# NoelShin/PixelPick

Hardware: AMD Instinct MI355X
Metric: train_step_throughput (higher is better)
Workload: dtype f32; 1 GPU; BASELINE configs[1]: Cityscapes 256x512, C=19, DeepLabv3+-MobileNetV2; train step per-GPU batch 4 with 20 labelled px/img + Adam; acquisition entropy top-k=20, B=256 images/launch/GPU, NCHW fp32 logits; global_batch=4

## Files before the change

### include/pixelpick_hip.h

```cpp
#ifndef PIXELPICK_HIP_H
#define PIXELPICK_HIP_H

#include <stddef.h>
#include <stdint.h>

#ifdef __cplusplus
extern "C" {
#endif

typedef void* pp_stream_t;

enum {
    PP_OK = 0,
    PP_ERR_BAD_ARG = -1,
    PP_ERR_BAD_K = -2,
    PP_ERR_WORKSPACE = -3,
    PP_ERR_UNSUPPORTED = -4,
    PP_ERR_LAUNCH = -5
};

enum { PP_ACQ_ENTROPY = 0, PP_ACQ_LEAST_CONFIDENCE = 1, PP_ACQ_MARGIN = 2 };
enum { PP_ACQ_BALD = 3 };
#define PP_ACQ_REFERENCE_ORDER 0x100

// ... 244 lines not shown

int pp_bn_eval_affine(int C, const float* gamma, const float* beta, const float* running_mean, const float* running_var,
                      float eps, float* scale, float* shift, pp_stream_t stream);

int pp_scale_shift_act(const float* x, int64_t ldx, int64_t M, int C, const float* scale, const float* shift,
                       const float* residual, int64_t ldr, int act, float* y, int64_t ldy, pp_stream_t stream);

int pp_bn_bwd(const float* x, int64_t ldx, const float* dy, int64_t lddy, const float* y_act, int64_t ldya, int act,
              int64_t M, int C, const float* mean, const float* invstd, const float* gamma, float* dgamma, float* dbeta,
              float* dx, int64_t lddx, float* dres, int64_t lddr, void* workspace, size_t ws_bytes, pp_stream_t stream);

int pp_dwconv3x3_fwd(const float* x, int64_t ldx, int B, int H, int W, int C, const float* w, int stride, int pad, int dil,
                     float* y, int64_t ldy, pp_stream_t stream);

int pp_dwconv3x3_fwd_bn_act(const float* x, int64_t ldx, int B, int H, int W, int C, const float* w, int stride, int pad,
                            int dil, const float* gamma, const float* beta, const float* running_mean,
                            const float* running_var, float eps, const float* residual, int64_t ldr, int act, float* y,
                            int64_t ldy, pp_stream_t stream);
int pp_dwconv3x3_bwd_data(const float* dy, int64_t lddy, int B, int H, int W, int C, const float* w, int stride, int pad,
                          int dil, float* dx, int64_t lddx, pp_stream_t stream);
int pp_dwconv3x3_bwd_weight(const float* x, int64_t ldx, int B, int H, int W, int C, const float* dy, int64_t lddy,
                            int stride, int pad, int dil, float* dw, void* workspace, size_t ws_bytes, pp_stream_t stream);

size_t pp_groupnorm_workspace_bytes(int B, int64_t P, int C);
int pp_groupnorm_relu_fwd(const float* x, int64_t ldx, int B, int64_t P, int C, int G, const float* gamma, const float* beta,
                          float eps, int relu, float* y, int64_t ldy, float* mean, float* rstd, void* workspace,
                          size_t ws_bytes, pp_stream_t stream);
int pp_groupnorm_relu_bwd(const float* x, int64_t ldx, const float* dy, int64_t lddy, const float* y, int64_t ldy, int B,
                          int64_t P, int C, int G, const float* mean, const float* rstd, const float* gamma, float* dgamma,
                          float* dbeta, float* dx, int64_t lddx, void* workspace, size_t ws_bytes, pp_stream_t stream);

int pp_maxpool2d_fwd(const float* x, int64_t ldx, int B, int H, int W, int C, int ksize, int stride, int pad, float* y,
                     int64_t ldy, unsigned char* argmax, pp_stream_t stream);
int pp_maxpool2d_bwd(const float* dy, int64_t lddy, const unsigned char* argmax, int B, int H, int W, int C, int ksize, int stride,
                     int pad, float* dx, int64_t lddx, pp_stream_t stream);

int pp_pad2d(const float* x, int64_t ldx, int B, int H, int W, int C, int pad_top, int pad_left, int Hp, int Wp, float* y,
             int64_t ldy, pp_stream_t stream);
int pp_crop2d_add(const float* xp, int64_t ldxp, int B, int Hp, int Wp, int C, int pad_top, int pad_left, const float* add,
                  int64_t ldadd, float* y, int64_t ldy, int H, int W, pp_stream_t stream);

int pp_bilinear_fwd(const float* x, int64_t ldx, int B, int H, int W, int C, float* y, int64_t ldy, int Ho, int Wo,
                    int align_corners, float scale_h, float scale_w, int out_nchw, pp_stream_t stream);
size_t pp_bilinear_bwd_workspace_bytes(int B, int Ho, int W, int C);
int pp_bilinear_bwd(const float* dy, int64_t lddy, int B, int Ho, int Wo, int C, float* dx, int64_t lddx, int H, int W,
                    int align_corners, float scale_h, float scale_w, int dy_nchw, void* workspace, size_t ws_bytes,
// ... 91 lines not shown
```

### include/pixelpick_hip_knobs.h

```cpp
#ifndef PIXELPICK_HIP_KNOBS_H
#define PIXELPICK_HIP_KNOBS_H

void pp_debug_set_reduce_mode(int mode);
void pp_debug_set_exact_formula(int on);
void pp_debug_set_acq_tuning(int occ, int ppt);
void pp_debug_set_dw_variant(int v);
void pp_debug_set_splitk(int v);
void pp_debug_set_wgrad_target(int blocks);
void pp_debug_set_bn_target(int blocks);
void pp_debug_set_bn_bytes_per_block(int bytes);
void pp_debug_set_bn_probe(void* device_buffer);
void pp_debug_set_lsel_probe(void* device_buffer);
void pp_debug_set_conv_thresholds(int v);
void pp_debug_conv_plan(int64_t M, int Cn, int Ck, int ntaps, int* out4);
void pp_debug_set_conv_rows(int bits);
void pp_debug_set_conv_bn_fuse(int bits);
void pp_debug_set_x3_variant(int v);
void pp_debug_set_gemm_pw(int v);
void pp_debug_set_x3f(int v);
void pp_debug_set_x3(int on);
void pp_debug_set_conv_variant(int v);
void pp_debug_set_ce_stream(int on);
int pp_debug_launch_log(char* buf, int n);


int pp_debug_occupy_cus(int blocks, const int* stop, uint64_t max_ticks, uint64_t* started, pp_stream_t stream);


#endif
```

### pixelpick_amd/_lib.py

```python
import ctypes
import os
import struct

import torch

_HERE = os.path.dirname(os.path.abspath(__file__))
LIB_PATH = os.path.join(_HERE, "libpixelpick_hip.so")
KNOBS_LIB_PATH = os.path.join(_HERE, "libpixelpick_hip_knobs.so")
_use_knobs = [os.environ.get("PIXELPICK_KNOBS_BUILD", "0") not in ("", "0")]


def use_knobs_build(on: bool = True):
    if _lib is not None and _use_knobs[0] != bool(on):
        raise PixelPickHipError("use_knobs_build() after the library was loaded")
    _use_knobs[0] = bool(on)


def knobs_build() -> bool:
    return _use_knobs[0]

_i64, _p, _int, _sz, _f = ctypes.c_int64, ctypes.c_void_p, ctypes.c_int, ctypes.c_size_t, ctypes.c_float
_u64 = ctypes.c_uint64

SIGNATURES = {
# ... 66 lines not shown
    "pp_conv2d_bwd_weight_pre": (_int, [_p, _i64, _int, _int, _int, _int, _p, _i64, _int, _int, _int, _int, _int, _int, _p, _p, _p, _sz, _p, _p, _p]),
    "pp_conv2d_bwd_weight_partials": (_int, [_p, _i64, _int, _int, _int, _int, _p, _i64, _int, _int, _int, _int, _int, _int, _p, _p, _p, _sz, _p, _p]),
    "pp_wgrad_reduce_batch": (_int, [_p, _int, _p]),
    "pp_colreduce_workspace_bytes": (_sz, [_i64, _int]),
    "pp_bn_train_fwd": (_int, [_p, _i64, _i64, _int, _p, _p, _f, _f, _p, _p, _p, _p, _p, _p, _p, _sz, _p]),
    "pp_bn_eval_affine": (_int, [_int, _p, _p, _p, _p, _f, _p, _p, _p]),
    "pp_scale_shift_act": (_int, [_p, _i64, _i64, _int, _p, _p, _p, _i64, _int, _p, _i64, _p]),
    "pp_bn_bwd": (_int, [_p, _i64, _p, _i64, _p, _i64, _int, _i64, _int, _p, _p, _p, _p, _p, _p, _i64, _p, _i64, _p, _sz, _p]),
    "pp_bn_fused_workspace_bytes": (_sz, [_i64, _int]),
    "pp_bn_fused_sync_ints": (_sz, [_int]),
    "pp_bn_fused_rows_cached": (_int, [_i64, _int]),
    "pp_bn_train_fwd_fused": (_int, [_p, _i64, _i64, _int, _p, _p, _f, _f, _p, _p, _p, _p, _p, _i64, _int, _f, _u64, _p, _p, _i64, _p, _sz, _p, _sz, _p]),
    "pp_dwconv3x3_bn_train_fwd_fused": (_int, [_p, _i64, _int, _int, _int, _int, _p, _int, _int, _int, _p, _i64, _p, _p, _f, _f, _p, _p, _p, _p,
                                               _p, _i64, _int, _p, _i64, _p, _sz, _p, _sz, _p]),
    "pp_bn_bwd_fused": (_int, [_p, _i64, _p, _i64, _p, _i64, _int, _i64, _int, _p, _p, _p, _p, _p, _p, _i64, _p, _i64, _f, _p, _p, _sz, _p, _sz, _p]),
    "pp_bn_bwd_fused_sparse": (_int, [_p, _i64, _p, _i64, _p, _i64, _int, _i64, _int, _p, _p, _p, _p, _p, _p, _i64, _p, _i64, _f, _p, _p, _sz, _p, _sz, _p, _p]),
    "pp_row_flags": (_int, [_p, _i64, _i64, _int, _p, _p]),
    "pp_conv1x1_bwd_weight_sparse_workspace_bytes": (_sz, [_i64, _int, _int]),
    "pp_conv1x1_bwd_weight_sparse": (_int, [_p, _i64, _i64, _int, _p, _i64, _int, _p, _p, _p, _p, _sz, _p]),
    "pp_conv1x1_bwd_data_sparse": (_int, [_p, _i64, _i64, _int, _p, _int, _p, _p, _i64, _p]),
    "pp_dwconv3x3_fwd": (_int, [_p, _i64, _int, _int, _int, _int, _p, _int, _int, _int, _p, _i64, _p]),
    "pp_dwconv3x3_bwd_data": (_int, [_p, _i64, _int, _int, _int, _int, _p, _int, _int, _int, _p, _i64, _p]),
    "pp_dwconv3x3_bwd_weight": (_int, [_p, _i64, _int, _int, _int, _int, _p, _i64, _int, _int, _int, _p, _p, _sz, _p]),
    "pp_dwconv3x3_bwd_weight_partials": (_int, [_p, _i64, _int, _int, _int, _int, _p, _i64, _int, _int, _int, _p, _p, _sz, _p, _p]),
    "pp_groupnorm_workspace_bytes": (_sz, [_int, _i64, _int]),
    "pp_groupnorm_relu_fwd": (_int, [_p, _i64, _int, _i64, _int, _int, _p, _p, _f, _int, _p, _i64, _p, _p, _p, _sz, _p]),
    "pp_groupnorm_relu_bwd": (_int, [_p, _i64, _p, _i64, _p, _i64, _int, _i64, _int, _int, _p, _p, _p, _p, _p, _p, _i64, _p, _sz, _p]),
    "pp_maxpool2d_fwd": (_int, [_p, _i64, _int, _int, _int, _int, _int, _int, _int, _p, _i64, _p, _p]),
    "pp_maxpool2d_bwd": (_int, [_p, _i64, _p, _int, _int, _int, _int, _int, _int, _int, _p, _i64, _p]),
    "pp_pad2d": (_int, [_p, _i64, _int, _int, _int, _int, _int, _int, _int, _int, _p, _i64, _p]),
    "pp_crop2d_add": (_int, [_p, _i64, _int, _int, _int, _int, _int, _int, _p, _i64, _p, _i64, _int, _int, _p]),
    "pp_bilinear_fwd": (_int, [_p, _i64, _int, _int, _int, _int, _p, _i64, _int, _int, _int, _f, _f, _int, _p]),
    "pp_bilinear_bwd_workspace_bytes": (_sz, [_int] * 4),
    "pp_bilinear_bwd": (_int, [_p, _i64, _int, _int, _int, _int, _p, _i64, _int, _int, _int, _f, _f, _int, _p, _sz, _p]),
    "pp_image_colsum": (_int, [_p, _i64, _int, _i64, _int, _f, _p, _i64, _p]),
    "pp_image_broadcast": (_int, [_p, _i64, _int, _i64, _int, _f, _p, _i64, _p]),
    "pp_dropout": (_int, [_p, _i64, _p, _i64, _i64, _int, _f, ctypes.c_uint64, _p, _p]),
    "pp_dropout2d": (_int, [_p, _i64, _p, _i64, _int, _i64, _int, _f, ctypes.c_uint64, _p, _p]),
    "pp_aug_resample_h": (_int, [_p, _int, _int, _p, _p, _int, _int, _p, _p]),
    "pp_aug_vcrop": (_int, [_p, _p, _p] + [_int] * 11 + [_p, _p]),
    "pp_aug_labels": (_int, [_p, _p, _int, _p, _p, _p, _p] + [_int] * 8 + [_p, _p, _p]),
    "pp_aug_jitter": (_int, [_p, _i64, _int, _f, _p, _p]),
    "pp_aug_blur": (_int, [_p, _int, _int, _p, _int, _p, _p]),
    "pp_aug_blur_q8": (_int, [_p, _int, _int, _p, _int, _p, _p]),
    "pp_aug_to_tensor": (_int, [_p, _i64, ctypes.POINTER(_f), ctypes.POINTER(_f), _p, _p]),
    "pp_sparse_ce_workspace_bytes": (_sz, []),
# ... 16 lines not shown
    "pp_set_kernel_events": (None, [_p, _p, _int]),
    "pp_set_comm_cu_reserve": (None, [_int]),
    "pp_get_comm_cu_reserve": (_int, []),
    "pp_plan_create": (_p, []),
    "pp_plan_destroy": (None, [_p]),
    "pp_plan_size": (_i64, [_p]),
    "pp_plan_entry_args": (_int, [_p]),
    "pp_plan_add_call": (_int, [_p, _p, _p, _int]),
    "pp_plan_add_event_record": (_int, [_p, _p, _p]),
    "pp_plan_add_stream_wait": (_int, [_p, _p, _p]),
    "pp_plan_add_join": (_int, [_p, _p, _p]),
    "pp_plan_add_host_break": (_int, [_p]),
    "pp_plan_replay": (_int, [_p, _i64, ctypes.POINTER(_i64)]),
}

KNOB_SIGNATURES = {
    "pp_debug_set_reduce_mode": (None, [_int]),
    "pp_debug_set_exact_formula": (None, [_int]),
    "pp_debug_set_acq_tuning": (None, [_int, _int]),
    "pp_debug_set_dw_variant": (None, [_int]),
    "pp_debug_set_splitk": (None, [_int]),
    "pp_debug_set_wgrad_target": (None, [_int]),
    "pp_debug_set_bn_target": (None, [_int]),
    "pp_debug_set_bn_bytes_per_block": (None, [_int]),
    "pp_debug_set_bn_probe": (None, [_p]),
    "pp_debug_set_lsel_probe": (None, [_p]),
    "pp_debug_set_conv_thresholds": (None, [_int]),
    "pp_debug_conv_plan": (None, [_i64, _int, _int, _int, _p]),
    "pp_debug_set_conv_variant": (None, [_int]),
    "pp_debug_set_ce_stream": (None, [_int]),
    "pp_debug_set_conv_rows": (None, [_int]),
    "pp_debug_set_conv_bn_fuse": (None, [_int]),
    "pp_debug_set_x3": (None, [_int]),
    "pp_debug_set_x3f": (None, [_int]),
    "pp_debug_set_gemm_pw": (None, [_int]),
    "pp_debug_set_x3_variant": (None, [_int]),
    "pp_debug_occupy_cus": (_int, [_int, _p, _u64, _p, _p]),
    "pp_debug_launch_log": (_int, [ctypes.c_char_p, _int]),
}

_lib = None
knob_epoch = [0]


def _knob_setter(fn):
    def setter(*args):
# ... 293 lines not shown
```

### pixelpick_amd/csrc/nn_ops.hip

```cpp
#include "pp_common.h"
#include "bn_xchg.h"
#include "lowres_tile.h"

namespace pp {

constexpr int kT = 256;

__device__ __forceinline__ float act_fwd(float z, int act)
{
    if (act == 1) return fmaxf(z, 0.0f);
    if (act == 2) return fminf(fmaxf(z, 0.0f), 6.0f);
    return z;
}
__device__ __forceinline__ void decode_bhwq(int64_t e, int cq, int Wd, int Hd, int& q, int& w, int& h, int& b)
{
    if (e <= 0xFFFFFFFFll) {
        const unsigned u = (unsigned)e;
        const unsigned t = u / (unsigned)cq;
        q = (int)(u - t * (unsigned)cq);
        const unsigned t2 = t / (unsigned)Wd;
        w = (int)(t - t2 * (unsigned)Wd);
        const unsigned t3 = t2 / (unsigned)Hd;
        h = (int)(t2 - t3 * (unsigned)Hd);
        b = (int)t3;
// ... 1107 lines not shown
                const int ih = 2 * ph + dr - pad, iw = 2 * pw + dc - pad;
                if ((unsigned)ih >= (unsigned)H || (unsigned)iw >= (unsigned)W) continue;
                float4 acc = make_float4(0.f, 0.f, 0.f, 0.f);
#pragma unroll
                for (int a = 0; a < 2; ++a) {
                    const int th = dr + 2 * a;
                    if (th > 2) continue;
                    const bool rok = (unsigned)(ph - a) < (unsigned)Ho;
#pragma unroll
                    for (int c = 0; c < 2; ++c) {
                        const int tw = dc + 2 * c;
                        if (tw > 2) continue;
                        if (!rok || (unsigned)(pw - c) >= (unsigned)Wo) continue;
                        const float4 gv = g[a][c], wv = ww[th * 3 + tw];
                        acc.x = fmaf(gv.x, wv.x, acc.x); acc.y = fmaf(gv.y, wv.y, acc.y);
                        acc.z = fmaf(gv.z, wv.z, acc.z); acc.w = fmaf(gv.w, wv.w, acc.w);
                    }
                }
                *reinterpret_cast<float4*>(dx + (((int64_t)b * H + ih) * W + iw) * lddx + q * 4) = acc;
            }
    }
}

__global__ __launch_bounds__(kT) void dwconv_bwd_weight_kernel(const float* x, int64_t ldx, int B, int H, int W, int cq,
                                                              const float* dy, int64_t lddy, int Ho, int Wo, int stride,
                                                              int pad, int dil, ColReduceGeom g, float* part,
                                                              const float* in_scale, const float* in_shift, int in_act)
{
    __shared__ float4 sh[kT];
    const int C = cq * 4;
    const int t = threadIdx.x;
    const int ql = t % g.cq_blk, ry = t / g.cq_blk;
    const int q = blockIdx.y * g.cq_blk + ql;
    const bool active = ry < g.rows_per_pass && q < cq;
    const int64_t M = (int64_t)B * Ho * Wo;
    float4 acc[9];
#pragma unroll
    for (int k = 0; k < 9; ++k) acc[k] = make_float4(0.f, 0.f, 0.f, 0.f);
    if (active) {
        const bool aff = in_scale != nullptr;
        float4 sc = make_float4(1.f, 1.f, 1.f, 1.f), sf = make_float4(0.f, 0.f, 0.f, 0.f);
        if (aff) { sc = *reinterpret_cast<const float4*>(in_scale + q * 4); sf = *reinterpret_cast<const float4*>(in_shift + q * 4); }
        const int64_t r0 = (int64_t)blockIdx.x * g.rows_per_block;
        const int64_t r1 = r0 + g.rows_per_block < M ? r0 + g.rows_per_block : M;
        for (int64_t r = r0 + ry; r < r1; r += g.rows_per_pass) {
            const unsigned ru = (unsigned)r;
// ... 901 lines not shown
        const float4 u = *reinterpret_cast<const float4*>(a + oa), v = *reinterpret_cast<const float4*>(b + ob);
        *reinterpret_cast<float4*>(y + oy) = make_float4(u.x + v.x, u.y + v.y, u.z + v.z, u.w + v.w);
    }
}

__global__ __launch_bounds__(kT) void nhwc_to_nchw_kernel(const float* x, int64_t ldx, int B, int C, int64_t HW, float* y)
{
    const int64_t total = (int64_t)B * C * HW;
    for (int64_t e = (int64_t)blockIdx.x * kT + threadIdx.x; e < total; e += (int64_t)gridDim.x * kT) {
        const int64_t pix = e % HW;
        const int64_t t = e / HW;
        const int c = (int)(t % C);
        const int64_t b = t / C;
        y[e] = x[(b * HW + pix) * ldx + c];
    }
}

static int g_ce_stream = 0;
static int g_bil_sep = 1;
static int g_dw_wgrad_x4 = 1, g_dw_wgrad_x4_blocks = 256;
static int g_dw_wgrad_cq_blk = 0, g_dw_wgrad_passes = 0;
static int g_dw_x4 = 1;
static int g_dw_s2 = 1;

static inline unsigned grid_for(int64_t total)
{
    int64_t b = cdiv(total, kT);
    if (b > 8192) b = 8192;
    if (b < 1) b = 1;
    return (unsigned)b;
}

static int need_c4(int C, const char* what)
{
    if (C < 4 || C % 4 != 0) return fail(PP_ERR_UNSUPPORTED, "%s: C=%d must be a positive multiple of 4", what, C);
    return PP_OK;
}

}

using namespace pp;

extern "C" {

#ifdef PP_DEBUG_KNOBS
void pp_debug_set_dw_variant(int v)
{
    g_dw_x4 = (v & 1) ? 0 : 1;
    g_dw_s2 = (v & 1048576) ? 0 : 1;
    g_bil_sep = (v & 256) ? 0 : 1;
    g_dw_wgrad_x4 = (v & 512) ? 0 : 1;
    { const int s4 = (v >> 10) & 7; g_dw_wgrad_x4_blocks = s4 == 1 ? 128 : s4 == 2 ? 512 : s4 == 3 ? 1024 : s4 == 4 ? 64 : 256; }
    { const int cb = (v >> 13) & 7; g_dw_wgrad_cq_blk = cb == 1 ? 8 : cb == 2 ? 16 : cb == 3 ? 32 : cb == 4 ? 64 : cb == 5 ? 128 : cb == 6 ? kT : 0; }
    { const int mp = (v >> 16) & 3; g_dw_wgrad_passes = mp == 1 ? 1 : mp == 2 ? 2 : mp == 3 ? 4 : 0; }
    const int sel = (v >> 1) & 7;
    g_dw_wgrad_blocks = sel == 1 ? 512 : sel == 2 ? 256 : sel == 3 ? 128 : sel == 4 ? 2048 : 1024;
}
#endif
#ifdef PP_DEBUG_KNOBS
void pp_debug_set_bn_target(int blocks) { g_bn_target_blocks = blocks > 0 ? (blocks > 1024 ? 1024 : blocks) : 0; }
#endif
#ifdef PP_DEBUG_KNOBS
void pp_debug_set_bn_bytes_per_block(int bytes)
{
    g_bn_bytes_per_block = bytes > 0 ? bytes : 0;
    g_bn_row_cache = bytes == -1 ? 0 : 1;
}
#endif
#ifdef PP_DEBUG_KNOBS
void pp_debug_set_ce_stream(int on) { g_ce_stream = on ? 1 : 0; }
#endif
static thread_local unsigned long long* g_bn_probe = nullptr;
#ifdef PP_DEBUG_KNOBS
void pp_debug_set_bn_probe(void* device_buffer) { g_bn_probe = reinterpret_cast<unsigned long long*>(device_buffer); }
#endif
int pp_bn_fused_capacity(void) { return bn_fused_capacity(); }

size_t pp_colreduce_workspace_bytes(int64_t M, int C)
{
    if (M < 1 || C < 4) return 256;
    ColReduceGeom g = col_geom(M, C);
    size_t a = (size_t)g.nblk_rows * 2 * C * 4;
    size_t b = (size_t)(M < 2048 ? M : 2048) * 9 * C * 4;
// ... 399 lines not shown
{
    if (!dy || !w || !dx) return fail(PP_ERR_BAD_ARG, "dwconv bwd_data: null");
    if (int rc = need_c4(C, "dwconv bwd_data")) return rc;
    const int Ho = (H + 2 * pad - 2 * dil - 1) / stride + 1, Wo = (W + 2 * pad - 2 * dil - 1) / stride + 1;
    if (stride == 1 && dil == 1 && g_dw_x4) {
        hipLaunchKernelGGL((dwconv_s1_x4_kernel<true>), dim3(grid_for((int64_t)B * H * ((W + 3) / 4) * (C / 4))), dim3(kT), 0,
                           as_stream(stream), dy, lddy, B, Ho, Wo, C / 4, w, 2 - pad, dx, lddx, H, W, Epilogue{});
        return check_launch("dwconv_s1_x4_kernel");
    }
    if (stride == 1 && dil == 2 && g_dw_x4) {
        hipLaunchKernelGGL((dwconv_s1_x4_kernel<true, 2>), dim3(grid_for((int64_t)B * H * ((W + 3) / 4) * (C / 4))), dim3(kT), 0,
                           as_stream(stream), dy, lddy, B, Ho, Wo, C / 4, w, 4 - pad, dx, lddx, H, W, Epilogue{});
        return check_launch("dwconv_s1_x4_kernel<2>");
    }
    if (stride == 2 && dil == 1 && pad >= 0 && pad <= 2 && g_dw_s2) {
        const int64_t items = (int64_t)B * ((H + pad + 1) / 2 + 1) * ((W + pad + 1) / 2 + 1) * (C / 4);
        hipLaunchKernelGGL(dwconv_s2_bwd_data_kernel, dim3(grid_for(items)), dim3(kT), 0, as_stream(stream), dy, lddy, B, Ho, Wo, C / 4, w, pad,
                           dx, lddx, H, W);
        return check_launch("dwconv_s2_bwd_data_kernel");
    }
    hipLaunchKernelGGL(dwconv_bwd_data_kernel, dim3(grid_for((int64_t)B * H * W * (C / 4))), dim3(kT), 0, as_stream(stream),
                       dy, lddy, B, Ho, Wo, C / 4, w, stride, pad, dil, dx, lddx, H, W);
    return check_launch("dwconv_bwd_data_kernel");
}

static int dwconv_bwd_weight_impl(const float* x, int64_t ldx, int B, int H, int W, int C, const float* dy, int64_t lddy,
                                  int stride, int pad, int dil, float* dw, void* workspace, size_t ws_bytes, pp_stream_t stream,
                                  const float* in_scale, const float* in_shift, int in_act, pp_reduce_job* job = nullptr)
{
    if (job) job->kind = 0;
    if (!x || !dy || !dw) return fail(PP_ERR_BAD_ARG, "dwconv bwd_weight: null");
    if (int rc = need_c4(C, "dwconv bwd_weight")) return rc;
    const int Ho = (H + 2 * pad - 2 * dil - 1) / stride + 1, Wo = (W + 2 * pad - 2 * dil - 1) / stride + 1;
    const int64_t M = (int64_t)B * Ho * Wo;
    if (M > 0x7FFFFFFFll) return fail(PP_ERR_UNSUPPORTED, "dwconv bwd_weight: more than 2^31 output pixels");
    if (!workspace || ws_bytes < pp_colreduce_workspace_bytes(M, C)) return fail(PP_ERR_WORKSPACE, "dwconv bwd_weight: workspace");
    const int cq_blk = g_dw_wgrad_cq_blk ? g_dw_wgrad_cq_blk : (M <= 8192 ? 32 : kT);
    const int passes = g_dw_wgrad_passes ? g_dw_wgrad_passes : (M <= 8192 ? 1 : 4);
    hipStream_t st = as_stream(stream);
    float* part = reinterpret_cast<float*>(workspace);
    if (stride == 1 && dil == 1 && Wo % 4 == 0 && g_dw_wgrad_x4) {
        ColReduceGeom g4 = col_geom(M / 4, C, g_dw_wgrad_x4_blocks, cq_blk, passes);
        if (g4.nblk_rows <= 2048) {
            hipLaunchKernelGGL(dwconv_bwd_weight_x4_kernel, dim3(g4.nblk_rows, g4.nblk_cols), dim3(kT), 0, st, x, ldx, B, H, W, C / 4,
                               dy, lddy, Ho, Wo, pad, g4, part, in_scale, in_shift, in_act);
            if (int rc = check_launch("dwconv_bwd_weight_x4_kernel")) return rc;
// ... 440 lines not shown
```

### pixelpick_amd/csrc/plan.hip

```cpp
#include "pp_common.h"

#include <cstring>
#include <type_traits>
#include <utility>
#include <vector>

namespace pp {
namespace {

template <typename T>
inline T unpack_slot(uint64_t s)
{
    if constexpr (std::is_same_v<T, float>) {
        float f;
        uint32_t lo = (uint32_t)s;
        memcpy(&f, &lo, 4);
        return f;
    } else if constexpr (std::is_same_v<T, double>) {
        double d;
        memcpy(&d, &s, 8);
        return d;
    } else if constexpr (std::is_pointer_v<T>) {
        return reinterpret_cast<T>(static_cast<uintptr_t>(s));
    } else {
// ... 57 lines not shown
    PP_PLAN_ENTRY(pp_x3_split),
    PP_PLAN_ENTRY(pp_conv2d_fwd_pre),
    PP_PLAN_ENTRY(pp_conv2d_bwd_data_pre),
    PP_PLAN_ENTRY(pp_conv2d_bwd_data_multi),
    PP_PLAN_ENTRY(pp_conv2d_fwd_pre2),
    PP_PLAN_ENTRY(pp_conv2d_bwd_data_pre2),
    PP_PLAN_ENTRY(pp_x3_split_weights),
    PP_PLAN_ENTRY(pp_conv2d_bwd_weight_pre),
    PP_PLAN_ENTRY(pp_conv2d_bwd_weight_partials),
    PP_PLAN_ENTRY(pp_wgrad_reduce_batch),
    PP_PLAN_ENTRY(pp_bn_train_fwd),
    PP_PLAN_ENTRY(pp_bn_eval_affine),
    PP_PLAN_ENTRY(pp_scale_shift_act),
    PP_PLAN_ENTRY(pp_bn_bwd),
    PP_PLAN_ENTRY(pp_bn_train_fwd_fused),
    PP_PLAN_ENTRY(pp_dwconv3x3_bn_train_fwd_fused),
    PP_PLAN_ENTRY(pp_bn_bwd_fused),
    PP_PLAN_ENTRY(pp_bn_bwd_fused_sparse),
    PP_PLAN_ENTRY(pp_row_flags),
    PP_PLAN_ENTRY(pp_conv1x1_bwd_weight_sparse),
    PP_PLAN_ENTRY(pp_conv1x1_bwd_data_sparse),
    PP_PLAN_ENTRY(pp_dwconv3x3_fwd),
    PP_PLAN_ENTRY(pp_dwconv3x3_bwd_data),
    PP_PLAN_ENTRY(pp_dwconv3x3_bwd_weight),
    PP_PLAN_ENTRY(pp_dwconv3x3_bwd_weight_partials),
    PP_PLAN_ENTRY(pp_groupnorm_relu_fwd),
    PP_PLAN_ENTRY(pp_groupnorm_relu_bwd),
    PP_PLAN_ENTRY(pp_maxpool2d_fwd),
    PP_PLAN_ENTRY(pp_maxpool2d_bwd),
    PP_PLAN_ENTRY(pp_pad2d),
    PP_PLAN_ENTRY(pp_crop2d_add),
    PP_PLAN_ENTRY(pp_bilinear_fwd),
    PP_PLAN_ENTRY(pp_bilinear_bwd),
    PP_PLAN_ENTRY(pp_image_colsum),
    PP_PLAN_ENTRY(pp_image_broadcast),
    PP_PLAN_ENTRY(pp_dropout),
    PP_PLAN_ENTRY(pp_dropout2d),
    PP_PLAN_ENTRY(pp_aug_resample_h),
    PP_PLAN_ENTRY(pp_aug_vcrop),
    PP_PLAN_ENTRY(pp_aug_labels),
    PP_PLAN_ENTRY(pp_aug_jitter),
    PP_PLAN_ENTRY(pp_aug_blur),
    PP_PLAN_ENTRY(pp_aug_blur_q8),
    PP_PLAN_ENTRY(pp_aug_to_tensor),
    PP_PLAN_ENTRY(pp_sparse_ce_fwd_bwd),
    PP_PLAN_ENTRY(pp_sparse_ce_lowres_fwd_bwd),
// ... 151 lines not shown
```

### pixelpick_amd/engine.py

```python
import contextlib
import math
import ctypes
import os
import weakref
from typing import List, Optional, Sequence

import torch

from . import _lib

ACT_NONE, ACT_RELU, ACT_RELU6 = 0, 1, 2


class Var:
    __slots__ = ("_t", "grad", "needs_grad", "_pending", "_lazy", "_bn_bwd_ctx", "_closed", "_grad_dst")

    def __init__(self, t: Optional[torch.Tensor], needs_grad: bool = True):
        self._t = t
        self.grad: Optional[torch.Tensor] = None
        self.needs_grad = needs_grad
        self._pending = None
        self._lazy = None
        self._bn_bwd_ctx = None
        self._closed = False
# ... 936 lines not shown
        if lazy_in is not None:
            raw, scale, shift, act = lazy_in
            with tape.side_stream_for(raw, dy, dw):
                ws = _ws(_wsbytes("pp_colreduce_workspace_bytes", B * Ho * Wo, C), dev)
                rc = L.pp_dwconv3x3_bwd_weight_affine_in(raw.data_ptr(), ldx, B, H, W, C, scale.data_ptr(), shift.data_ptr(), act,
                                                         dy.data_ptr(), lddy, stride, pad, dil, dw.data_ptr(), ws.data_ptr(), ws.numel(),
                                                         _stream())
            _lib.check(rc, "pp_dwconv3x3_bwd_weight_affine_in")
        else:
            with tape.side_stream_for(x.t, dy, dw):
                nws = _wsbytes("pp_colreduce_workspace_bytes", B * Ho * Wo, C)
                slot = tape.defer_slot(nws, dev)
                if slot is not None:
                    job, wptr, _ = slot
                    rc = L.pp_dwconv3x3_bwd_weight_partials(x.t.data_ptr(), ldx, B, H, W, C, dy.data_ptr(), lddy, stride, pad, dil,
                                                            dw.data_ptr(), wptr, nws, ctypes.addressof(job), _stream())
                    tape.defer_commit(job)
                else:
                    ws = _ws(nws, dev)
                    rc = L.pp_dwconv3x3_bwd_weight(x.t.data_ptr(), ldx, B, H, W, C, dy.data_ptr(), lddy, stride, pad, dil, dw.data_ptr(),
                                                   ws.data_ptr(), ws.numel(), _stream())
            _lib.check(rc, "pp_dwconv3x3_bwd_weight")
        tape.set_param_grad(w, dw)
    if x.needs_grad:
        dx = torch.empty((B, H, W, C), dtype=torch.float32, device=dev)
        rc = L.pp_dwconv3x3_bwd_data(dy.data_ptr(), lddy, B, H, W, C, w.data_ptr(), stride, pad, dil, dx.data_ptr(), C, _stream())
        _lib.check(rc, "pp_dwconv3x3_bwd_data")
        _acc(x, dx)


def _dw_bn_train_fused(tape: Tape, x: Var, gamma, beta, running_mean, running_var, act, residual, eps, momentum, dst):
    _, xin, w, _, stride, pad, dil = x._pending
    B, H, W, C, ld_in = _geom(xin.t)
    Ho, Wo = out_size(H, 3, stride, pad, dil), out_size(W, 3, stride, pad, dil)
    M = B * Ho * Wo
    if M > _BN_FUSED_MAXM or M >= (1 << 31) or C > 65536 or C % 4 or ld_in % 4:
        return None
    dev = xin.t.device
    xbuf = torch.empty((B, Ho, Wo, C), dtype=torch.float32, device=dev)
    mean = torch.empty(C, dtype=torch.float32, device=dev)
    invstd = torch.empty(C, dtype=torch.float32, device=dev)
    y = dst if dst is not None else torch.empty((B, Ho, Wo, C), dtype=torch.float32, device=dev)
    _, _, _, _, ldy = _geom(y)
    rptr, ldr = (None, 0)
    if residual is not None:
        _, _, _, _, ldr = _geom(residual.t)
        rptr = residual.t.data_ptr()
# ... 6 lines not shown
    _lib.check(rc, "pp_dwconv3x3_bn_train_fwd_fused")
    x._pending = None
    x._t = xbuf
    out = Var(y)
    tape.record(_bn_bwd, (x, gamma, beta, mean, invstd, act, residual, out, 1.0), out)
    return out


_CONV_BN_STATS_MAX_ROWS = int(os.environ.get("PIXELPICK_CONV_BN_STATS_MAX_ROWS", "160"))


_CONV_BN_FUSE = os.environ.get("PIXELPICK_CONV_BN_FUSE", "1") != "0"


def _conv_bn_fusable(B, H, W, Cin, Cout, kh, kw, stride, pad, dil) -> bool:
    if not (_BN_FUSED and Cout % 32 == 0):
        return False
    if not _wsbytes("pp_conv2d_fwd_bn_train_ok", B, H, W, Cin, Cout, kh, kw, stride, pad, dil):
        return False
    return _wsbytes("pp_conv2d_fwd_bn_train_xchg_bytes", B, H, W, Cin, Cout, kh, kw, stride, pad, dil) <= _BN_XCHG_PART_BYTES


_CONV_BN_FUSE_BWD = os.environ.get("PIXELPICK_CONV_BN_FUSE_BWD", "1") != "0"
_SPARSE_ROWS = os.environ.get("PIXELPICK_SPARSE_ROWS", "1") != "0"
_WGRAD_LATE = os.environ.get("PIXELPICK_WGRAD_LATE", "0") != "0"
_SPARSE_WGRAD = os.environ.get("PIXELPICK_SPARSE_WGRAD", "1") != "0"


def _conv_bn_bwd_fusable(B, H, W, Cin, Cout, kh, kw, stride, pad, dil) -> bool:
    if not (_BN_FUSED and Cin % 32 == 0):
        return False
    if not _wsbytes("pp_conv2d_bwd_data_bn_bwd_ok", B, H, W, Cin, Cout, kh, kw, stride, pad, dil):
        return False
    return _wsbytes("pp_conv2d_bwd_data_bn_bwd_xchg_bytes", B, H, W, Cin, Cout, kh, kw, stride, pad, dil) <= _BN_XCHG_PART_BYTES


def _conv_bn_train_fused(tape: Tape, x: Var, gamma, beta, running_mean, running_var, act, residual, eps, momentum, dst, ncons=0):
    _, xin, w, bias, stride, pad, dil = x._pending
    if bias is not None:
        return None
    B, H, W, Cin, ldx = _geom(xin.t)
    kh, kw, _, Cout = w.shape
    if not _conv_bn_fusable(B, H, W, Cin, Cout, kh, kw, stride, pad, dil) or ldx % 4:
        return None
    if (xin.t.data_ptr() | w.data_ptr()) & 15:
        return None
# ... 574 lines not shown
```

### pixelpick_amd/profiling.py

```python
import ctypes
from typing import Callable, Dict, List, Optional

import torch


def _ival(a) -> int:
    return int(a.value) if isinstance(a, ctypes._SimpleCData) and a.value is not None else 0


_DW_GEOM = {
    "pp_dwconv3x3_fwd": ((2, 3, 4, 5), (7, 8, 9)),
    "pp_dwconv3x3_fwd_fused": ((2, 3, 4, 5), (7, 8, 9)),
    "pp_dwconv3x3_bn_train_fwd_fused": ((2, 3, 4, 5), (7, 8, 9)),
    "pp_dwconv3x3_bwd_data": ((2, 3, 4, 5), (7, 8, 9)),
    "pp_dwconv3x3_bwd_weight": ((2, 3, 4, 5), (8, 9, 10)),
    "pp_dwconv3x3_bwd_weight_partials": ((2, 3, 4, 5), (8, 9, 10)),
    "pp_dwconv3x3_bwd_weight_affine_in": ((2, 3, 4, 5), (11, 12, 13)),
}


def depthwise_calls(plan) -> List[Dict]:
    out = []
    for i, (fn, args) in enumerate(plan.calls):
        name = getattr(fn, "__name__", "")
        if name not in _DW_GEOM:
            continue
        (ib, ih, iw, ic), (isd, ipd, idl) = _DW_GEOM[name]
        B, H, W, C = (_ival(args[j]) for j in (ib, ih, iw, ic))
        s, p, d = (_ival(args[j]) for j in (isd, ipd, idl))
        Ho, Wo = (H + 2 * p - 2 * d - 1) // s + 1, (W + 2 * p - 2 * d - 1) // s + 1
        s_in, s_out = 4 * B * H * W * C, 4 * B * Ho * Wo * C
        if name == "pp_dwconv3x3_bwd_data":
            kind, read, write = "bwd_data", s_out, s_in
        elif "bwd_weight" in name:
            kind, read, write = "bwd_weight", s_in + s_out, 0
        else:
            kind, read, write = "fwd", s_in, s_out
            if name == "pp_dwconv3x3_bn_train_fwd_fused":
                write += s_out
        out.append({"index": i, "entry": name, "kind": kind, "B": B, "H": H, "W": W, "C": C, "stride": s, "pad": p, "dil": d,
                    "Ho": Ho, "Wo": Wo, "read_bytes": read, "write_bytes": write, "fn": fn, "args": args})
    return out


def time_call(fn: Callable, args, iters: int = 20, flush: Optional[torch.Tensor] = None, cold: bool = False) -> float:
    ts = []
    for _ in range(iters):
        if cold:
            flush.zero_()
        else:
            assert fn(*args) == 0
        a, b = torch.cuda.Event(enable_timing=True), torch.cuda.Event(enable_timing=True)
        a.record()
        rc = fn(*args)
        b.record()
        assert rc == 0, getattr(fn, "__name__", fn)
# ... 28 lines not shown
                c["yardstick"] = "read-only kernel over x + dy bytes"
            else:
                src = torch.empty(c["read_bytes"] // 4, device=dev).normal_()
                dst = torch.empty(c["write_bytes"] // 4, device=dev)
                n = min(src.numel(), dst.numel())
                extra = src.numel() - n

                def yfn(_s=src, _d=dst, _n=n, _e=extra):
                    _d[:_n].copy_(_s[:_n])
                    if _e > 0:
                        L.pp_yardstick_stream_read(_s[_n:].data_ptr(), _e * 4 // 16 * 16, -256, sink.data_ptr(), torch.cuda.current_stream().cuda_stream)
                    return 0
                c["yardstick"] = "torch copy (+ read-only kernel for the unread rest)" if extra > 0 else "torch copy of the same bytes"
            c["yard_us_warm"] = round(time_call(yfn, (), iters), 2)
            if with_cold:
                c["yard_us_cold"] = round(time_call(yfn, (), max(iters // 2, 5), flush, True), 2)
            c["x_yardstick_warm"] = round(c["us_warm"] / c["yard_us_warm"], 2)
        rows.append(c)
    return rows


def depthwise_summary(rows: List[Dict], large_bytes: int = 16 << 20) -> Dict:
    out = {}
    for kind in ("fwd", "bwd_data", "bwd_weight"):
        rs = [r for r in rows if r["kind"] == kind]
        if not rs:
            continue
        by = sum(r["read_bytes"] + r["write_bytes"] for r in rs)
        us = sum(r["us_warm"] for r in rs)
        big = [r for r in rs if r["read_bytes"] + r["write_bytes"] >= large_bytes]
        worst = min(big, key=lambda r: r["TBps_warm"]) if big else None
        out[kind] = {"launches": len(rs), "bytes_per_step": by, "us_per_step_warm": round(us, 1), "TBps_warm": round(by / us / 1e6, 3),
                     "frac_of_8TBps": round(by / us / 1e6 / 8.0, 4),
                     "large_layers_TBps_warm": [r["TBps_warm"] for r in big],
                     "worst_large_layer": ({k: worst[k] for k in ("entry", "H", "W", "C", "stride", "us_warm", "TBps_warm")} if worst else None)}
    return out
```

Baseline: 762.7 images/s.

## Fuse depthwise conv backward-data with preceding BatchNorm backward for stride-2 layers

Adds a fused kernel pair that recomputes the depthwise 3x3 input gradient on the fly, reduces the BatchNorm dgamma/dbeta statistics from it, then recomputes it again to apply the BN input gradient. The engine routes large stride-2, pad-0 depthwise layers whose input comes straight from a BatchNorm (no residual, no dropout) through this path. This avoids writing and rereading the intermediate dx tensor between the conv backward and the BN backward, at the cost of running the depthwise gather twice and doing the reductions in doubles.

```diff
diff --git a/include/pixelpick_hip.h b/include/pixelpick_hip.h
--- a/include/pixelpick_hip.h
+++ b/include/pixelpick_hip.h
@@ -290,6 +290,12 @@
 int pp_dwconv3x3_bwd_weight(const float* x, int64_t ldx, int B, int H, int W, int C, const float* dy, int64_t lddy,
                             int stride, int pad, int dil, float* dw, void* workspace, size_t ws_bytes, pp_stream_t stream);
 
+size_t pp_dwconv3x3_bwd_data_bn_bwd_workspace_bytes(int B, int H, int W, int C);
+int pp_dwconv3x3_bwd_data_bn_bwd(const float* dyo, int64_t lddyo, int B, int H, int W, int C, const float* w, int stride, int pad, int dil,
+                                 const float* bn_x, int64_t ldbx, const float* mean, const float* invstd, const float* gamma,
+                                 const float* beta, int act, float* dgamma, float* dbeta, float* dx_bn, int64_t lddx, float* dres,
+                                 float grad_scale, void* workspace, size_t ws_bytes, pp_stream_t stream);
+
 size_t pp_groupnorm_workspace_bytes(int B, int64_t P, int C);
 int pp_groupnorm_relu_fwd(const float* x, int64_t ldx, int B, int64_t P, int C, int G, const float* gamma, const float* beta,
                           float eps, int relu, float* y, int64_t ldy, float* mean, float* rstd, void* workspace,
diff --git a/include/pixelpick_hip_knobs.h b/include/pixelpick_hip_knobs.h
--- a/include/pixelpick_hip_knobs.h
+++ b/include/pixelpick_hip_knobs.h
@@ -8,6 +8,7 @@
 void pp_debug_set_splitk(int v);
 void pp_debug_set_wgrad_target(int blocks);
 void pp_debug_set_bn_target(int blocks);
+void pp_debug_set_dw_bn_bwd_blocks(int blocks);
 void pp_debug_set_bn_bytes_per_block(int bytes);
 void pp_debug_set_bn_probe(void* device_buffer);
 void pp_debug_set_lsel_probe(void* device_buffer);
diff --git a/pixelpick_amd/_lib.py b/pixelpick_amd/_lib.py
--- a/pixelpick_amd/_lib.py
+++ b/pixelpick_amd/_lib.py
@@ -112,6 +112,9 @@
     "pp_dwconv3x3_fwd": (_int, [_p, _i64, _int, _int, _int, _int, _p, _int, _int, _int, _p, _i64, _p]),
     "pp_dwconv3x3_bwd_data": (_int, [_p, _i64, _int, _int, _int, _int, _p, _int, _int, _int, _p, _i64, _p]),
     "pp_dwconv3x3_bwd_weight": (_int, [_p, _i64, _int, _int, _int, _int, _p, _i64, _int, _int, _int, _p, _p, _sz, _p]),
+    "pp_dwconv3x3_bwd_data_bn_bwd_workspace_bytes": (_sz, [_int] * 4),
+    "pp_dwconv3x3_bwd_data_bn_bwd": (_int, [_p, _i64, _int, _int, _int, _int, _p, _int, _int, _int, _p, _i64, _p, _p, _p, _p, _int, _p, _p, _p, _i64,
+                                            _p, _f, _p, _sz, _p]),
     "pp_dwconv3x3_bwd_weight_partials": (_int, [_p, _i64, _int, _int, _int, _int, _p, _i64, _int, _int, _int, _p, _p, _sz, _p, _p]),
     "pp_groupnorm_workspace_bytes": (_sz, [_int, _i64, _int]),
     "pp_groupnorm_relu_fwd": (_int, [_p, _i64, _int, _i64, _int, _int, _p, _p, _f, _int, _p, _i64, _p, _p, _p, _sz, _p]),
@@ -174,6 +177,7 @@
     "pp_debug_set_splitk": (None, [_int]),
     "pp_debug_set_wgrad_target": (None, [_int]),
     "pp_debug_set_bn_target": (None, [_int]),
+    "pp_debug_set_dw_bn_bwd_blocks": (None, [_int]),
     "pp_debug_set_bn_bytes_per_block": (None, [_int]),
     "pp_debug_set_bn_probe": (None, [_p]),
     "pp_debug_set_lsel_probe": (None, [_p]),
diff --git a/pixelpick_amd/csrc/nn_ops.hip b/pixelpick_amd/csrc/nn_ops.hip
--- a/pixelpick_amd/csrc/nn_ops.hip
+++ b/pixelpick_amd/csrc/nn_ops.hip
@@ -1153,6 +1153,166 @@
     }
 }
 
+template <int S>
+__device__ __forceinline__ float4 dw_bwd_g(const float* dyq , int64_t lddy, int b, int ih, int iw, int Ho, int Wo, int pad,
+                                           const float4* ww)
+{
+    float4 acc = make_float4(0.f, 0.f, 0.f, 0.f);
+    if constexpr (S == 1) {
+        const int pf = 2 - pad;
+#pragma unroll
+        for (int th = 0; th < 3; ++th) {
+            const int oh = ih - pf + th;
+            if ((unsigned)oh >= (unsigned)Ho) continue;
+            const float* row = dyq + ((int64_t)b * Ho + oh) * Wo * lddy;
+            float4 v[3];
+#pragma unroll
+            for (int tw = 0; tw < 3; ++tw) {
+                const int ow = iw - pf + tw;
+                v[tw] = (unsigned)ow < (unsigned)Wo ? *reinterpret_cast<const float4*>(row + (int64_t)ow * lddy) : make_float4(0.f, 0.f, 0.f, 0.f);
+            }
+#pragma unroll
+            for (int tw = 0; tw < 3; ++tw) {
+                const float4 wk = ww[(2 - th) * 3 + (2 - tw)];
+                acc.x = fmaf(v[tw].x, wk.x, acc.x); acc.y = fmaf(v[tw].y, wk.y, acc.y);
+                acc.z = fmaf(v[tw].z, wk.z, acc.z); acc.w = fmaf(v[tw].w, wk.w, acc.w);
+            }
+        }
+    } else {
+        const int ph = (ih + pad) >> 1, dr = (ih + pad) & 1, pw = (iw + pad) >> 1, dc = (iw + pad) & 1;
+        float4 g[2][2];
+        bool ok[2][2];
+#pragma unroll
+        for (int a = 0; a < 2; ++a)
+#pragma unroll
+            for (int c = 0; c < 2; ++c) {
+                const int oh = ph - a, ow = pw - c;
+                ok[a][c] = dr + 2 * a <= 2 && dc + 2 * c <= 2 && (unsigned)oh < (unsigned)Ho && (unsigned)ow < (unsigned)Wo;
+                g[a][c] = *reinterpret_cast<const float4*>(dyq + (ok[a][c] ? (((int64_t)b * Ho + oh) * Wo + ow) * lddy : 0));
+            }
+        auto sel = [](int c, float4 p, float4 n) { return make_float4(c ? p.x : n.x, c ? p.y : n.y, c ? p.z : n.z, c ? p.w : n.w); };
+        const float4 wsel[2][2] = {{sel(dr, sel(dc, ww[4], ww[3]), sel(dc, ww[1], ww[0])), sel(dr, ww[5], ww[2])}, {sel(dc, ww[7], ww[6]), ww[8]}};
+#pragma unroll
+        for (int a = 0; a < 2; ++a)
+#pragma unroll
+            for (int c = 0; c < 2; ++c) {
+                const float4 wk = wsel[a][c];
+                if (ok[a][c]) {
+                    acc.x = fmaf(g[a][c].x, wk.x, acc.x); acc.y = fmaf(g[a][c].y, wk.y, acc.y);
+                    acc.z = fmaf(g[a][c].z, wk.z, acc.z); acc.w = fmaf(g[a][c].w, wk.w, acc.w);
+                }
+            }
+    }
+    return acc;
+}
+
+__device__ __forceinline__ float4 bn_remask(float4 g, float4 v, float4 zsc, float4 zsf, int act)
+{
+    if (act != 0) {
+        g.x *= act_mask(fmaf(v.x, zsc.x, zsf.x), act); g.y *= act_mask(fmaf(v.y, zsc.y, zsf.y), act);
+        g.z *= act_mask(fmaf(v.z, zsc.z, zsf.z), act); g.w *= act_mask(fmaf(v.w, zsc.w, zsf.w), act);
+    }
+    return g;
+}
+
+struct DwBnBwdArgs {
+    const float* dyo; int64_t lddyo; int B, H, W, Ho, Wo, cq, pad;
+    const float* w; const float* x; int64_t ldx; const float* mean; const float* invstd; const float* gamma; const float* beta; int act;
+};
+
+template <int S>
+__global__ __launch_bounds__(kT) void dw_bn_bwd_stats_kernel(DwBnBwdArgs a, int64_t M, ColReduceGeom g, float* part )
+{
+    __shared__ double sh[2][4][kT];
+    const int C = a.cq * 4;
+    const int t = threadIdx.x;
+    const int ql = t % g.cq_blk, ry = t / g.cq_blk;
+    const int q = blockIdx.y * g.cq_blk + ql;
+    const bool active = ry < g.rows_per_pass && q < a.cq;
+    double d0[4] = {0.0, 0.0, 0.0, 0.0}, d1[4] = {0.0, 0.0, 0.0, 0.0};
+    if (active) {
+        float4 ww[9];
+#pragma unroll
+        for (int k = 0; k < 9; ++k) ww[k] = *reinterpret_cast<const float4*>(a.w + k * C + q * 4);
+        const float4 mu = *reinterpret_cast<const float4*>(a.mean + q * 4), is = *reinterpret_cast<const float4*>(a.invstd + q * 4);
+        float4 zsc = make_float4(0.f, 0.f, 0.f, 0.f), zsf = zsc;
+        if (a.act != 0) {
+            const float4 gm = *reinterpret_cast<const float4*>(a.gamma + q * 4), be = *reinterpret_cast<const float4*>(a.beta + q * 4);
+            zsc = make_float4(gm.x * is.x, gm.y * is.y, gm.z * is.z, gm.w * is.w);
+            zsf = make_float4(be.x - mu.x * zsc.x, be.y - mu.y * zsc.y, be.z - mu.z * zsc.z, be.w - mu.w * zsc.w);
+        }
+        const float* dyq = a.dyo + q * 4;
+        const int64_t r0 = (int64_t)blockIdx.x * g.rows_per_block;
+        const int64_t r1 = r0 + g.rows_per_block < M ? r0 + g.rows_per_block : M;
+#pragma unroll 2
+        for (int64_t r = r0 + ry; r < r1; r += g.rows_per_pass) {
+            const unsigned ru = (unsigned)r;
+            const unsigned tt = ru / (unsigned)a.W;
+            const int iw = (int)(ru - tt * (unsigned)a.W);
+            const int b = (int)(tt / (unsigned)a.H);
+            const int ih = (int)(tt - (unsigned)b * (unsigned)a.H);
+            const float4 v = *reinterpret_cast<const float4*>(a.x + r * a.ldx + q * 4);
+            const float4 gg = bn_remask(dw_bwd_g<S>(dyq, a.lddyo, b, ih, iw, a.Ho, a.Wo, a.pad, ww), v, zsc, zsf, a.act);
+            d0[0] += (double)gg.x; d0[1] += (double)gg.y; d0[2] += (double)gg.z; d0[3] += (double)gg.w;
+            d1[0] += (double)gg.x * (double)((v.x - mu.x) * is.x); d1[1] += (double)gg.y * (double)((v.y - mu.y) * is.y);
+            d1[2] += (double)gg.z * (double)((v.z - mu.z) * is.z); d1[3] += (double)gg.w * (double)((v.w - mu.w) * is.w);
+        }
+    }
+#pragma unroll
+    for (int j = 0; j < 4; ++j) { sh[0][j][t] = d0[j]; sh[1][j][t] = d1[j]; }
+    __syncthreads();
+    if (ry == 0 && q < a.cq) {
+        for (int k = 1; k < g.rows_per_pass; ++k) {
+#pragma unroll
+            for (int j = 0; j < 4; ++j) { d0[j] += sh[0][j][k * g.cq_blk + ql]; d1[j] += sh[1][j][k * g.cq_blk + ql]; }
+        }
+        *reinterpret_cast<float4*>(part + ((int64_t)blockIdx.x * 2 + 0) * C + q * 4) = make_float4((float)d0[0], (float)d0[1], (float)d0[2], (float)d0[3]);
+        *reinterpret_cast<float4*>(part + ((int64_t)blockIdx.x * 2 + 1) * C + q * 4) = make_float4((float)d1[0], (float)d1[1], (float)d1[2], (float)d1[3]);
+    }
+}
+
+template <int S>
+__global__ __launch_bounds__(kT) void dw_bn_bwd_apply_kernel(DwBnBwdArgs a, int64_t M, ColReduceGeom g, const float* dgamma,
+                                                            const float* dbeta, float inv_count, float* dx, int64_t lddx)
+{
+    const int C = a.cq * 4;
+    const int t = threadIdx.x;
+    const int ql = t % g.cq_blk, ry = t / g.cq_blk;
+    const int q = blockIdx.y * g.cq_blk + ql;
+    if (ry >= g.rows_per_pass || q >= a.cq) return;
+    float4 ww[9];
+#pragma unroll
+    for (int k = 0; k < 9; ++k) ww[k] = *reinterpret_cast<const float4*>(a.w + k * C + q * 4);
+    const float4 mu = *reinterpret_cast<const float4*>(a.mean + q * 4), is = *reinterpret_cast<const float4*>(a.invstd + q * 4);
+    const float4 ga = *reinterpret_cast<const float4*>(a.gamma + q * 4);
+    const float4 dg = *reinterpret_cast<const float4*>(dgamma + q * 4), db = *reinterpret_cast<const float4*>(dbeta + q * 4);
+    float4 zsc = make_float4(0.f, 0.f, 0.f, 0.f), zsf = zsc;
+    if (a.act != 0) {
+        const float4 be = *reinterpret_cast<const float4*>(a.beta + q * 4);
+        zsc = make_float4(ga.x * is.x, ga.y * is.y, ga.z * is.z, ga.w * is.w);
+        zsf = make_float4(be.x - mu.x * zsc.x, be.y - mu.y * zsc.y, be.z - mu.z * zsc.z, be.w - mu.w * zsc.w);
+    }
+    const float* dyq = a.dyo + q * 4;
+    const int64_t r0 = (int64_t)blockIdx.x * g.rows_per_block;
+    const int64_t r1 = r0 + g.rows_per_block < M ? r0 + g.rows_per_block : M;
+#pragma unroll 2
+    for (int64_t r = r0 + ry; r < r1; r += g.rows_per_pass) {
+        const unsigned ru = (unsigned)r;
+        const unsigned tt = ru / (unsigned)a.W;
+        const int iw = (int)(ru - tt * (unsigned)a.W);
+        const int b = (int)(tt / (unsigned)a.H);
+        const int ih = (int)(tt - (unsigned)b * (unsigned)a.H);
+        const float4 v = *reinterpret_cast<const float4*>(a.x + r * a.ldx + q * 4);
+        const float4 u = bn_remask(dw_bwd_g<S>(dyq, a.lddyo, b, ih, iw, a.Ho, a.Wo, a.pad, ww), v, zsc, zsf, a.act);
+        float4 o;
+        o.x = bn_dx(u.x, v.x, mu.x, is.x, ga.x, db.x, dg.x, inv_count);
+        o.y = bn_dx(u.y, v.y, mu.y, is.y, ga.y, db.y, dg.y, inv_count);
+        o.z = bn_dx(u.z, v.z, mu.z, is.z, ga.z, db.z, dg.z, inv_count);
+        o.w = bn_dx(u.w, v.w, mu.w, is.w, ga.w, db.w, dg.w, inv_count);
+        *reinterpret_cast<float4*>(dx + r * lddx + q * 4) = o;
+    }
+}
+
 __global__ __launch_bounds__(kT) void dwconv_bwd_weight_kernel(const float* x, int64_t ldx, int B, int H, int W, int cq,
                                                               const float* dy, int64_t lddy, int Ho, int Wo, int stride,
                                                               int pad, int dil, ColReduceGeom g, float* part,
@@ -2100,6 +2260,9 @@
 static int g_dw_wgrad_cq_blk = 0, g_dw_wgrad_passes = 0;
 static int g_dw_x4 = 1;
 static int g_dw_s2 = 1;
+constexpr int kDwBnBwdStatBlocks = 1024, kDwBnBwdApplyBlocks = 8192;
+static int g_dw_bn_bwd_blocks = 0;
+static ColReduceGeom dw_bn_bwd_stat_geom(int64_t M, int C) { return col_geom(M, C, g_dw_bn_bwd_blocks > 0 ? g_dw_bn_bwd_blocks : kDwBnBwdStatBlocks); }
 
 static inline unsigned grid_for(int64_t total)
 {
@@ -2137,6 +2300,7 @@
 #endif
 #ifdef PP_DEBUG_KNOBS
 void pp_debug_set_bn_target(int blocks) { g_bn_target_blocks = blocks > 0 ? (blocks > 1024 ? 1024 : blocks) : 0; }
+void pp_debug_set_dw_bn_bwd_blocks(int blocks) { g_dw_bn_bwd_blocks = blocks > 0 ? (blocks > 8192 ? 8192 : blocks) : 0; }
 #endif
 #ifdef PP_DEBUG_KNOBS
 void pp_debug_set_bn_bytes_per_block(int bytes)
@@ -2582,6 +2746,58 @@
     hipLaunchKernelGGL(dwconv_bwd_data_kernel, dim3(grid_for((int64_t)B * H * W * (C / 4))), dim3(kT), 0, as_stream(stream),
                        dy, lddy, B, Ho, Wo, C / 4, w, stride, pad, dil, dx, lddx, H, W);
     return check_launch("dwconv_bwd_data_kernel");
+}
+
+size_t pp_dwconv3x3_bwd_data_bn_bwd_workspace_bytes(int B, int H, int W, int C)
+{
+    if (B < 1 || H < 1 || W < 1 || C < 4) return 256;
+    const int64_t M = (int64_t)B * H * W;
+    const int64_t rows = M < 8192 ? M : 8192;
+    return align_up((size_t)rows * 2 * (size_t)C * 4, 256);
+}
+
+int pp_dwconv3x3_bwd_data_bn_bwd(const float* dyo, int64_t lddyo, int B, int H, int W, int C, const float* w, int stride, int pad, int dil,
+                                 const float* bn_x, int64_t ldbx, const float* mean, const float* invstd, const float* gamma,
+                                 const float* beta, int act, float* dgamma, float* dbeta, float* dx_bn, int64_t lddx, float* dres,
+                                 float grad_scale, void* workspace, size_t ws_bytes, pp_stream_t stream)
+{
+    const char* what = "dwconv bwd_data + BatchNorm bwd";
+    if (!dyo || !w || !bn_x || !mean || !invstd || !gamma || !dgamma || !dbeta || !dx_bn) return fail(PP_ERR_BAD_ARG, "%s: null", what);
+    if (dres) return fail(PP_ERR_BAD_ARG, "%s: a BatchNorm with a residual is not served (pp_dwconv3x3_bwd_data + pp_bn_bwd_fused)", what);
+    if (grad_scale != 1.0f) return fail(PP_ERR_BAD_ARG, "%s: a BatchNorm with a fused dropout is not served", what);
+    if (act < 0 || act > 2) return fail(PP_ERR_BAD_ARG, "%s: act %d", what, act);
+    if (act != 0 && !beta) return fail(PP_ERR_BAD_ARG, "%s: the mask needs beta", what);
+    if (B < 1 || H < 1 || W < 1) return fail(PP_ERR_BAD_ARG, "%s: empty map", what);
+    if (C < 4 || C % 4 != 0) return fail(PP_ERR_BAD_ARG, "%s: C=%d must be a positive multiple of 4", what, C);
+    if (!(dil == 1 && ((stride == 1 && (pad == 0 || pad == 1)) || (stride == 2 && pad == 0))))
+        return fail(PP_ERR_BAD_ARG, "%s: stride %d pad %d dil %d (served: stride 1 pad 0/1, stride 2 pad 0, dil 1)", what, stride, pad, dil);
+    const int Ho = (H + 2 * pad - 3) / stride + 1, Wo = (W + 2 * pad - 3) / stride + 1;
+    if (H + 2 * pad < 3 || W + 2 * pad < 3 || Ho < 1 || Wo < 1) return fail(PP_ERR_BAD_ARG, "%s: empty convolution output", what);
+    const int64_t M = (int64_t)B * H * W;
+    if (M >= (1ll << 31)) return fail(PP_ERR_BAD_ARG, "%s: %lld pixels", what, (long long)M);
+    if (lddyo % 4 || ldbx % 4 || lddx % 4 || lddyo < C || ldbx < C || lddx < C) return fail(PP_ERR_BAD_ARG, "%s: pixel strides %lld / %lld / %lld must be multiples of 4, >= C", what, (long long)lddyo, (long long)ldbx, (long long)lddx);
+    if (((uintptr_t)dyo | (uintptr_t)w | (uintptr_t)bn_x | (uintptr_t)mean | (uintptr_t)invstd | (uintptr_t)gamma | (uintptr_t)beta |
+         (uintptr_t)dgamma | (uintptr_t)dbeta | (uintptr_t)dx_bn | (uintptr_t)workspace) & 15)
+        return fail(PP_ERR_BAD_ARG, "%s: pointers must be 16-byte aligned", what);
+    if (!workspace || ws_bytes < pp_dwconv3x3_bwd_data_bn_bwd_workspace_bytes(B, H, W, C)) return fail(PP_ERR_WORKSPACE, "%s: workspace", what);
+    const ColReduceGeom g1 = dw_bn_bwd_stat_geom(M, C), g2 = col_geom(M, C, kDwBnBwdApplyBlocks);
+    const DwBnBwdArgs a{dyo, lddyo, B, H, W, Ho, Wo, C / 4, pad, w, bn_x, ldbx, mean, invstd, gamma, beta, act};
+    float* part = reinterpret_cast<float*>(workspace);
+    hipStream_t st = as_stream(stream);
+    if (stride == 1)
+        hipLaunchKernelGGL(dw_bn_bwd_stats_kernel<1>, dim3(g1.nblk_rows, g1.nblk_cols), dim3(kT), 0, st, a, M, g1, part);
+    else
+        hipLaunchKernelGGL(dw_bn_bwd_stats_kernel<2>, dim3(g1.nblk_rows, g1.nblk_cols), dim3(kT), 0, st, a, M, g1, part);
+    if (int rc = check_launch("dw_bn_bwd_stats_kernel")) return rc;
+    hipLaunchKernelGGL(bn_bwd_finalize_kernel, dim3((unsigned)cdiv(C, 8)), dim3(kT), 0, st, part, g1.nblk_rows, C, dgamma, dbeta);
+    if (int rc = check_launch("bn_bwd_finalize_kernel")) return rc;
+    if (stride == 1)
+        hipLaunchKernelGGL(dw_bn_bwd_apply_kernel<1>, dim3(g2.nblk_rows, g2.nblk_cols), dim3(kT), 0, st, a, M, g2, dgamma, dbeta,
+                           1.0f / (float)M, dx_bn, lddx);
+    else
+        hipLaunchKernelGGL(dw_bn_bwd_apply_kernel<2>, dim3(g2.nblk_rows, g2.nblk_cols), dim3(kT), 0, st, a, M, g2, dgamma, dbeta,
+                           1.0f / (float)M, dx_bn, lddx);
+    return check_launch("dw_bn_bwd_apply_kernel");
 }
 
 static int dwconv_bwd_weight_impl(const float* x, int64_t ldx, int B, int H, int W, int C, const float* dy, int64_t lddy,
diff --git a/pixelpick_amd/csrc/plan.hip b/pixelpick_amd/csrc/plan.hip
--- a/pixelpick_amd/csrc/plan.hip
+++ b/pixelpick_amd/csrc/plan.hip
@@ -103,6 +103,7 @@
     PP_PLAN_ENTRY(pp_conv1x1_bwd_data_sparse),
     PP_PLAN_ENTRY(pp_dwconv3x3_fwd),
     PP_PLAN_ENTRY(pp_dwconv3x3_bwd_data),
+    PP_PLAN_ENTRY(pp_dwconv3x3_bwd_data_bn_bwd),
     PP_PLAN_ENTRY(pp_dwconv3x3_bwd_weight),
     PP_PLAN_ENTRY(pp_dwconv3x3_bwd_weight_partials),
     PP_PLAN_ENTRY(pp_groupnorm_relu_fwd),
diff --git a/pixelpick_amd/engine.py b/pixelpick_amd/engine.py
--- a/pixelpick_amd/engine.py
+++ b/pixelpick_amd/engine.py
@@ -982,7 +982,28 @@
                                                    ws.data_ptr(), ws.numel(), _stream())
             _lib.check(rc, "pp_dwconv3x3_bwd_weight")
         tape.set_param_grad(w, dw)
-    if x.needs_grad:
+    bctx = x._bn_bwd_ctx if (x.needs_grad and _DW_BN_BWD_MIN_BYTES is not None and lazy_in is None and not x._closed) else None
+    if (bctx is not None and bctx[7] == 1 and x.grad is None and bctx[6] is None and bctx[0].needs_grad
+            and 4 * B * H * W * C >= _DW_BN_BWD_MIN_BYTES and dil == 1 and (stride, pad) == (2, 0) and C % 4 == 0
+            and lddy % 4 == 0 and B * H * W < (1 << 31) and _geom(bctx[0].t)[4] % 4 == 0
+            and not ((dy.data_ptr() | w.data_ptr() | bctx[0].t.data_ptr() | bctx[1].data_ptr() | bctx[2].data_ptr()) & 15)):
+        bin_, g_, b_, mean_, invstd_, act_, _, _ = bctx
+        _, _, _, _, ldb = _geom(bin_.t)
+        dxbn = torch.empty((B, H, W, C), dtype=torch.float32, device=dev)
+        dg_, db_ = tape.grad_buffer_for(g_), tape.grad_buffer_for(b_)
+        nws = _wsbytes("pp_dwconv3x3_bwd_data_bn_bwd_workspace_bytes", B, H, W, C)
+        ws = _ws(nws, dev)
+        rc = L.pp_dwconv3x3_bwd_data_bn_bwd(dy.data_ptr(), lddy, B, H, W, C, w.data_ptr(), stride, pad, dil, bin_.t.data_ptr(), ldb,
+                                            mean_.data_ptr(), invstd_.data_ptr(), g_.data_ptr(), b_.data_ptr(), act_, dg_.data_ptr(),
+                                            db_.data_ptr(), dxbn.data_ptr(), C, None, 1.0, ws.data_ptr(), ws.numel(), _stream())
+        _lib.check(rc, "pp_dwconv3x3_bwd_data_bn_bwd")
+        tape.set_param_grad(g_, dg_)
+        tape.set_param_grad(b_, db_)
+        x.grad = None
+        x._closed = True
+        dxbn._pp_owned = True
+        _acc(bin_, dxbn)
+    elif x.needs_grad:
         dx = torch.empty((B, H, W, C), dtype=torch.float32, device=dev)
         rc = L.pp_dwconv3x3_bwd_data(dy.data_ptr(), lddy, B, H, W, C, w.data_ptr(), stride, pad, dil, dx.data_ptr(), C, _stream())
         _lib.check(rc, "pp_dwconv3x3_bwd_data")
@@ -1035,6 +1056,8 @@
 
 
 _CONV_BN_FUSE_BWD = os.environ.get("PIXELPICK_CONV_BN_FUSE_BWD", "1") != "0"
+_DW_BN_BWD_MIN_BYTES = os.environ.get("PIXELPICK_DW_BN_BWD_MIN_BYTES", str(18 << 20))
+_DW_BN_BWD_MIN_BYTES = None if _DW_BN_BWD_MIN_BYTES.lower() == "off" else int(_DW_BN_BWD_MIN_BYTES)
 _SPARSE_ROWS = os.environ.get("PIXELPICK_SPARSE_ROWS", "1") != "0"
 _WGRAD_LATE = os.environ.get("PIXELPICK_WGRAD_LATE", "0") != "0"
 _SPARSE_WGRAD = os.environ.get("PIXELPICK_SPARSE_WGRAD", "1") != "0"
diff --git a/pixelpick_amd/profiling.py b/pixelpick_amd/profiling.py
--- a/pixelpick_amd/profiling.py
+++ b/pixelpick_amd/profiling.py
@@ -13,6 +13,7 @@
     "pp_dwconv3x3_fwd_fused": ((2, 3, 4, 5), (7, 8, 9)),
     "pp_dwconv3x3_bn_train_fwd_fused": ((2, 3, 4, 5), (7, 8, 9)),
     "pp_dwconv3x3_bwd_data": ((2, 3, 4, 5), (7, 8, 9)),
+    "pp_dwconv3x3_bwd_data_bn_bwd": ((2, 3, 4, 5), (7, 8, 9)),
     "pp_dwconv3x3_bwd_weight": ((2, 3, 4, 5), (8, 9, 10)),
     "pp_dwconv3x3_bwd_weight_partials": ((2, 3, 4, 5), (8, 9, 10)),
     "pp_dwconv3x3_bwd_weight_affine_in": ((2, 3, 4, 5), (11, 12, 13)),
@@ -32,6 +33,8 @@
         s_in, s_out = 4 * B * H * W * C, 4 * B * Ho * Wo * C
         if name == "pp_dwconv3x3_bwd_data":
             kind, read, write = "bwd_data", s_out, s_in
+        elif name == "pp_dwconv3x3_bwd_data_bn_bwd":
+            kind, read, write = "bwd_data_bn", s_out + s_in, s_in
         elif "bwd_weight" in name:
             kind, read, write = "bwd_weight", s_in + s_out, 0
         else:
@@ -106,7 +109,7 @@
 
 def depthwise_summary(rows: List[Dict], large_bytes: int = 16 << 20) -> Dict:
     out = {}
-    for kind in ("fwd", "bwd_data", "bwd_weight"):
+    for kind in ("fwd", "bwd_data", "bwd_data_bn", "bwd_weight"):
         rs = [r for r in rows if r["kind"] == kind]
         if not rs:
             continue
```

Result: no change. 765.8 images/s, median of 6 (+0.4%).
